# christoskokas/gtsam-vSLAM

Measured on AMD Instinct MI355X. Metric: frames/sec (extract+match+localBA), 1500 feat stereo 752x480, higher is better.
Workload: dtype u8/i32 (extract, match) + f64 (pose LM, local BA)

## Files before the change

### gtsam-vslam_amd/csrc/ba.hip

```cpp
#include "common.hpp"
#include "comm.hpp"
#include "dmath.hpp"
#include "ba_pool.hpp"
#include <algorithm>
#include <cmath>
#include <numeric>
#include <vector>
#include <atomic>
#include <condition_variable>
#include <functional>
#include <memory>
#include <mutex>
#include <thread>

namespace vslam {

struct BaEdge {
    int a, b, fa, fb;
    DPose measured;
    double r[6], Ja[36], Jb[36];
    double Haa[36], Hab[36], Hbb[36], ga[6], gb[6];
};

struct BaDev {
    int NF, Lp, F, K, NE, n;
    const int* facKf; const int* facFi; const int* facLp; const int* facLm;
    const double* facZ; const double* facIs; const uint8_t* facRight;
    double* facJ;
    const int* lpStart; const int* lpSlotStart; const int* slotStart; const int* slotFi; const int* lpOrig;
    DPose* poseCur; DPose* poseTrial; const int* fidx;
    double* lmCur; double* lmTrial;
    BaEdge* edges;
    double* S; double* rhs; double* Spart; double* Sedge; double* dP; double* dL;
    double* sums; double* partial;
    int* flags;
    double fx, fy, cx, cy, b;
// ... 557 lines not shown
        const double2* src = (const double2*)(D.facJ + (size_t)f0 * 20);
        double2* dst = (double2*)g.F;
        for (int i = lane; i < nf * 10; i += 64) dst[i] = src[i];
        for (int i = lane; i < nf; i += 64) g.ffi[i] = D.facFi[f0 + i];
        for (int i = lane; i <= ns; i += 64) { g.sst[i] = D.slotStart[s0 + i] - f0; g.sfi[i] = D.slotFi[s0 + i]; }
    }
    ba_wave_fence();
    {
        double acc = 0;
        if (R.hOn)
            for (int f = R.hq; f < nf; f += 4) {
                const double* o = g.F + f * 20;
                acc += o[R.hx] * o[R.hy] + o[R.hx + 3] * o[R.hy + R.hyStep];
            }
        acc += ba2_dpp_xor(acc, 0);
        acc += ba2_dpp_xor(acc, 1);
        if (R.hOn && R.hq == 0) g.hb[R.hk] = R.hSign * acc;
    }
    ba_wave_fence();
#pragma unroll
    for (int k = 0; k < 9; k++) h[k] = g.hb[k];
}
__device__ __forceinline__ void ba2_w_row(const Ba2Region& g, const Ba2Roles& R, double& w0, double& w1, double& w2) {
    w0 = w1 = w2 = 0;
    for (int f = g.sst[R.ws]; f < g.sst[R.ws + 1]; f++) {
        const double* o = g.F + f * 20;
        const double a0 = o[2 + R.wi], a1 = o[8 + R.wi];
        w0 += a0 * o[14] + a1 * o[17];
        w1 += a0 * o[15] + a1 * o[18];
        w2 += a0 * o[16] + a1 * o[19];
    }
}

__global__ __launch_bounds__(1024) void k_ba_schur2(const BaDev* __restrict__ tab, int maxSlots, int maxFac) {
    BaDev D = *lane_entry(tab, blockIdx.z);
    extern __shared__ double sm[];
    if (!ba_enter(D, BA_TRY, blockIdx.y)) return;
    const int n = D.n;
    const int sys = n * n + n;
    double* const Sloc = sm;
    double* const racc = Sloc + (size_t)n * n;
    const int lane = threadIdx.x & 63;
    const int unit = __builtin_amdgcn_readfirstlane(threadIdx.x >> 6), nu = blockDim.x >> 6, nt = blockDim.x;
    const Ba2Region g = ba2_region(sm + sys + (size_t)unit * ba2_stage_doubles(maxFac, maxSlots), maxFac, maxSlots);
    double* const F = g.F; double* const W = g.W; double* const WH = g.WH;
    int* const ffi = g.ffi; int* const sfi = g.sfi;
    const double lam = D.lambda;
    Ba2Roles R;
    R.init(lane);
    const int pf = lane / 6, pi = lane - pf * 6;
    for (int i = threadIdx.x; i < sys; i += nt) Sloc[i] = 0;
    __syncthreads();
    for (int lp = blockIdx.x * nu + unit; lp < D.Lp; lp += gridDim.x * nu) {
        double h[9];
        int nf, ns;
        ba2_stage_h(D, lp, g, R, lane, h, nf, ns);
        double Hi[9];
        ba_hll_inverse(h, lam, Hi);
        if (R.ws < ns) {
            double w0, w1, w2;
            ba2_w_row(g, R, w0, w1, w2);
            const double g0 = w0 * Hi[0] + w1 * Hi[3] + w2 * Hi[6], g1 = w0 * Hi[1] + w1 * Hi[4] + w2 * Hi[7], g2 = w0 * Hi[2] + w1 * Hi[5] + w2 * Hi[8];
            double* wr = W + R.ws * 18 + R.wi * 3;
            wr[0] = w0; wr[1] = w1; wr[2] = w2;
            double* gr = WH + R.ws * 18 + R.wi * 3;
            gr[0] = g0; gr[1] = g1; gr[2] = g2;
            atomicAdd(&racc[6 * sfi[R.ws] + R.wi], -(g0 * h[6] + g1 * h[7] + g2 * h[8]));
        }
        ba_wave_fence();
        {
            const int nb = ns * (ns + 1) / 2, half = lane & 1;
            for (int b0 = 0; b0 < nb; b0 += 32) {
                int b = b0 + (lane >> 1), s1 = 0;
                if (b >= nb) continue;
                while (b >= ns - s1) { b -= ns - s1; s1++; }
                const int s2 = s1 + b;
                const double* A = WH + s1 * 18 + half * 9;
                const double* B = W + s2 * 18;
                double bb[18];
#pragma unroll
                for (int q = 0; q < 18; q++) bb[q] = B[q];
                double* d0 = Sloc + (6 * sfi[s1] + 3 * half) * n + 6 * sfi[s2];
#pragma unroll
                for (int i = 0; i < 3; i++) {
                    const double a0 = A[3 * i], a1 = A[3 * i + 1], a2 = A[3 * i + 2];
                    double* dr = d0 + i * n;
#pragma unroll
                    for (int j = 0; j < 6; j++) atomicAdd(dr + j, -(a0 * bb[3 * j] + a1 * bb[3 * j + 1] + a2 * bb[3 * j + 2]));
                }
            }
        }
        if (pf < 10)
            for (int fb = 0; fb < nf; fb += 10) {
                const int f = fb + pf;
                if (f >= nf) break;
                const int fi = ffi[f];
                if (fi < 0) continue;
                const double* o = F + f * 20;
                const double a0 = o[2 + pi], a1 = o[8 + pi];
                double* dr = Sloc + (6 * fi + pi) * n + 6 * fi;
                for (int j = pi; j < 6; j++) atomicAdd(dr + j, a0 * o[2 + j] + a1 * o[8 + j]);
                atomicAdd(&racc[6 * fi + pi], -(a0 * o[0] + a1 * o[1]));
            }
        ba_wave_fence();
    }
    __syncthreads();
    double* dst = D.Spart + (size_t)blockIdx.x * sys;
    for (int i = threadIdx.x; i < sys; i += nt) dst[i] = Sloc[i];
}

__global__ __launch_bounds__(512) void k_ba_back2(const BaDev* __restrict__ tab, int maxSlots, int maxFac) {
    BaDev D = *lane_entry(tab, blockIdx.z);
    extern __shared__ double sm[];
    if (!ba_enter(D, BA_TRY, 0)) return;
    const int nc = D.nAct;
    const int sel = ((const int*)(D.ctl + CTL_INTS))[CI_SEL];
    const int lane = threadIdx.x & 63;
    const int unit = __builtin_amdgcn_readfirstlane(threadIdx.x >> 6), nu = blockDim.x >> 6;
    const Ba2Region g = ba2_region(sm + (size_t)unit * ba2_stage_doubles(maxFac, maxSlots), maxFac, maxSlots);
    Ba2Roles R;
    R.init(lane);
    for (int lp = blockIdx.x * nu + unit; lp < D.Lp; lp += gridDim.x * nu) {
        double h[9];
        int nf, ns;
        ba2_stage_h(D, lp, g, R, lane, h, nf, ns);
        double w0 = 0, w1 = 0, w2 = 0;
        int kcol = 0;
        if (R.ws < ns) { ba2_w_row(g, R, w0, w1, w2); kcol = 6 * g.sfi[R.ws] + R.wi; }
        const int l = D.lpOrig[lp];
        double lamk = D.lambda;
        for (int k = 0; k < nc; k++, lamk *= 10.0) {
            const double* dPk = D.dP + (size_t)k * D.n;
            const double dp = R.ws < ns ? dPk[kcol] : 0.0;
            double t0 = w0 * dp, t1 = w1 * dp, t2 = w2 * dp;
            t0 += ba2_dpp_xor(t0, 0); t1 += ba2_dpp_xor(t1, 0); t2 += ba2_dpp_xor(t2, 0);
            t0 += ba2_dpp_xor(t0, 1); t1 += ba2_dpp_xor(t1, 1); t2 += ba2_dpp_xor(t2, 1);
#pragma unroll
            for (int d = 4; d <= 32; d <<= 1) { t0 += __shfl_xor(t0, d); t1 += __shfl_xor(t1, d); t2 += __shfl_xor(t2, d); }
            double Hi[9];
            ba_hll_inverse(h, lamk, Hi);
            if (lane < 3) {
                const double u0 = h[6] - t0, u1 = h[7] - t1, u2 = h[8] - t2;
                const double h0 = lane == 0 ? Hi[0] : (lane == 1 ? Hi[3] : Hi[6]);
                const double h1 = lane == 0 ? Hi[1] : (lane == 1 ? Hi[4] : Hi[7]);
                const double h2 = lane == 0 ? Hi[2] : (lane == 1 ? Hi[5] : Hi[8]);
                const double dl = h0 * u0 + h1 * u1 + h2 * u2;
                D.dL[(size_t)k * D.dLStride + 3 * (size_t)lp + lane] = dl;
                double* lmT = D.lmBase + (size_t)ba_slot(sel, k, D.NB) * D.lmStride;
                lmT[3 * (size_t)l + lane] = D.lmCur[3 * (size_t)l + lane] + dl;
            }
        }
        ba_wave_fence();
    }
}

__global__ __launch_bounds__(256) void k_ba_reduce(const BaDev* __restrict__ tab, int nPart) {
    BaDev D = *lane_entry(tab, blockIdx.z);
    __shared__ double sSl[8][33];
    if (!ba_enter(D, BA_TRY, blockIdx.y)) return;
    const int total = D.n * D.n + D.n;
    const int e = threadIdx.x & 31, y = threadIdx.x >> 5;
    const int i = blockIdx.x * 32 + e;
    const size_t stride = (size_t)total;
    double s = 0;
    if (i < total) {
        const int per = (nPart + 7) / 8;
        const int p0 = y * per, p1 = min(nPart, p0 + per);
        double s0 = 0, s1 = 0, s2 = 0, s3 = 0;
        int p = p0;
        for (; p + 3 < p1; p += 4) {
            s0 += D.Spart[(size_t)p * stride + i];
            s1 += D.Spart[(size_t)(p + 1) * stride + i];
            s2 += D.Spart[(size_t)(p + 2) * stride + i];
            s3 += D.Spart[(size_t)(p + 3) * stride + i];
        }
        for (; p < p1; p++) s0 += D.Spart[(size_t)p * stride + i];
        s = (s0 + s1) + (s2 + s3);
    }
    sSl[y][e] = s;
    __syncthreads();
    if (y == 0 && i < total) {
        double t = D.Sedge[i];
        for (int q = 0; q < 8; q++) t += sSl[q][e];
        if (D.specLin) D.Sedge2[i] = 0;
        if (i < D.n * D.n) D.S[i] = t; else D.rhs[i - D.n * D.n] = t;
    }
}

struct BaWin {
    int TB, T, TP, tileDoubles, nWin;
    const int* winA; const int* winB;
    const int* winFirstWg;
    const int* wgWin; const int* wgBegin; const int* wgEnd;
    const int* winLm;
    double* part;
    double* Wg; double* Hg;
};

constexpr int BA_WIN_HG = 9 + 6 * BA_MAX_NB;
__global__ __launch_bounds__(64 * BA_SCHUR_WAVES) void k_ba_lm_prep(const BaDev* __restrict__ tab, BaWin Wn, int maxSlots) {
    BaDev D = *lane_entry(tab, blockIdx.z);
    extern __shared__ int smi[];
    if (!ba_enter(D, BA_TRY, 0)) return;
    constexpr int BA_LPL = 64;
    const int lane = threadIdx.x & 63, unit = threadIdx.x >> 6, nu = blockDim.x >> 6;
    int* sfi = smi + unit * maxSlots;
    for (int lp = blockIdx.x * nu + unit; lp < D.Lp; lp += gridDim.x * nu) {
        double h[9];
        int ns = 0;
        ba_lm_blocks<BA_LPL>(D, lp, true, Wn.Wg + (size_t)D.lpSlotStart[lp] * 18, sfi, h, ns);
        double* Hl = Wn.Hg + (size_t)lp * BA_WIN_HG;
        if (lane < 9) {
            double v = h[0];
#pragma unroll
            for (int k = 1; k < 9; k++) if (lane == k) v = h[k];
            Hl[lane] = v;
        } else if (lane >= 16 && lane < 16 + D.nAct) {
            double lamk = D.lambda;
// ... 1557 lines not shown
                    h_facIs[f] = 1.0 / (1.0 / (double)P->inv_sigma_factor[P->pair_octave[2 * p + side]]);
                    h_facRight[f] = (uint8_t)side;
                    h_facPair[f] = p;
                }
                h_slotStart[se] = f1; h_slotFi[se] = -1;
            }
        });
        h_lpSlotStart[Lp] = nSlotEntries;
        for (int l = 0; l < L; l++) h_lmPresent[l] = T.lmPresent[l];
        fill_small(P, T, pose0, edgeSlots);
    }
    void fill_small(const vslam_ba_problem* P, BaHostTmp& T, const DPose* pose0, int edgeSlots) {
        const int K = P->n_kf;
        for (int k = 0; k < K; k++) { h_fidx[k] = T.fidx[k]; h_kfPresent[k] = T.kfPresent[k]; }
        for (int i = 0; i < NE; i++) {
            BaEdge e{};
            e.a = T.order[i]; e.b = T.order[i + 1]; e.fa = T.fidx[e.a]; e.fb = T.fidx[e.b];
            DPose ai;
            pose_inverse(pose0[e.a], ai);
            pose_compose(ai, pose0[e.b], e.measured);
            for (int sl = 0; sl < edgeSlots; sl++) h_edges[(size_t)sl * NE + i] = e;
        }
    }
};

static vslam_status ba_kernel_attributes() {
    static std::once_flag once;
    static hipError_t err = hipSuccess;
    static bool reserveOk = true;
    std::call_once(once, [] {
        const int cap = BA_LDS_BYTES;
        const void* fns[] = {(const void*)k_ba_schur, (const void*)k_ba_schur_win, (const void*)k_ba_solve, (const void*)k_ba_back,
                             (const void*)k_ba_solve_mfma, (const void*)k_ba_chol_col, (const void*)k_ba_chol_back, (const void*)k_ba_lm_prep,
                             (const void*)k_ba_schur2, (const void*)k_ba_back2};
        const void* batchFns[] = {(const void*)k_ba_schur, (const void*)k_ba_schur2, (const void*)k_ba_back, (const void*)k_ba_back2, (const void*)k_ba_solve_mfma};
        for (const void* f : fns) {
            hipFuncAttributes fa{};
            hipError_t e = hipFuncGetAttributes(&fa, f);
            if (e == hipSuccess) e = hipFuncSetAttribute(f, hipFuncAttributeMaxDynamicSharedMemorySize, cap - (int)fa.sharedSizeBytes);
            if (e != hipSuccess && err == hipSuccess) err = e;
            for (const void* b : batchFns) if (b == f && e == hipSuccess && fa.sharedSizeBytes > (size_t)BA_STATIC_LDS_RESERVE) reserveOk = false;
        }
    });
    if (err != hipSuccess) { set_error("hipFuncSetAttribute(MaxDynamicSharedMemorySize): %s", hipGetErrorString(err)); return VSLAM_ERR_HIP; }
    if (!reserveOk) { set_error("local BA: a batch kernel's static LDS exceeds BA_STATIC_LDS_RESERVE"); return VSLAM_ERR_CAPACITY; }
    return VSLAM_OK;
}

static vslam_status ba_run(const vslam_ba_problem* P, vslam_ba_result* R, int device, const vslam_comm* comm) {
#ifdef VSLAM_HOST_STAMPS
    const double bhs_fn0 = bhs_now();
#endif
#ifndef VSLAM_HOST_STAMPS
    auto bhs_t = std::chrono::steady_clock::now();
    g_bhsCalls++;
#endif
    if (!P || !R || P->n_kf < 1 || P->n_lm < 0 || P->n_pairs < 0 || P->n_levels < 1 || P->n_levels > MAX_LEVELS ||
        !P->kf_pose_wc || !P->kf_id || !P->kf_fixed || !P->kf_local || !P->sigma_factor || !P->inv_sigma_factor ||
        !R->kf_pose_wc || !R->lm_xyz || !R->pair_wrong ||
        (P->n_lm > 0 && !P->lm_xyz) ||
        (P->n_pairs > 0 && (!P->pair_kf || !P->pair_lm || !P->pair_flags || !P->pair_uv || !P->pair_octave))) {
        set_error("vslam_local_ba: invalid problem");
        return VSLAM_ERR_INVALID;
    }
    const int rank = comm ? comm->rank : 0, world = comm ? comm->world : 1;
    int ndev = 0;
    if (hipGetDeviceCount(&ndev) != hipSuccess || ndev <= 0) { set_error("no HIP device available (no CPU fallback)"); return VSLAM_ERR_NO_DEVICE; }
    if (device < 0 || device >= ndev) return VSLAM_ERR_INVALID;
// ... 461 lines not shown
        const BaDev* const dD = A.dev(h_D);
        VS_HIP(hipMemcpyAsync((void*)dD, h_D, sizeof(BaDev), hipMemcpyHostToDevice, stream));
        BHS("upload");

        auto run_lm = [&](int ps, long long nfStat, long long lpStat, long long k2Stat) -> vslam_status {
        (void)poseOut; (void)lmOut;
        const int fuseCtl = comm ? 0 : 1;
        const int facBlocks = (NF ? obsBlocks : 0) + std::max(NE, 1);
        const int nObs = NF ? obsBlocks : 0;
        VS_HIP(hipMemsetAsync(d_Sedge.p, 0, ((size_t)n * n + n) * sizeof(double), stream));
        auto step = [&](bool first) -> vslam_status {
            int t = -1;
            if (first || !specLin) {
                t = g_baTimer.begin("ba_linearize");
                hipLaunchKernelGGL(k_ba_factors<0>, dim3(facBlocks), dim3(256), 0, stream, dD, nObs, fuseCtl, relTol, absTol);
                g_baTimer.end(t);
            }
            if (comm) {
                const int tc = g_baTimer.begin("ba_allreduce"); VS_CHECK(comm_allreduce(comm, d_sums.p, 1, stream)); g_baTimer.end(tc);
                hipLaunchKernelGGL(k_ba_ctl, dim3(1), dim3(256), 0, stream, dD, 0, relTol, absTol);
            }
            t = g_baTimer.begin("ba_schur");
            if (n > 0) {
                if (ldsS) hipLaunchKernelGGL(k_ba_schur, dim3(lmBlocks, sharedW ? 1 : NB), dim3(64 * schurWaves), schurLds, stream, dD, maxSlots, sharedW);
                else if (nWinWg) {
                    hipLaunchKernelGGL(k_ba_lm_prep, dim3(std::max(1, std::min((Lp + BA_SCHUR_WAVES - 1) / BA_SCHUR_WAVES, 4 * nCU))), dim3(64 * BA_SCHUR_WAVES),
                                       (size_t)BA_SCHUR_WAVES * maxSlots * sizeof(int), stream, dD, Wn, maxSlots);
                    hipLaunchKernelGGL(k_ba_schur_win, dim3(nWinWg), dim3(64 * schurWaves), schurLds, stream, dD, Wn);
                }
            }
            g_baTimer.end(t);
            t = g_baTimer.begin("ba_solve");
            if (n > 0) {
                if (ldsS) hipLaunchKernelGGL(k_ba_reduce, dim3(((int)sysDoubles + 31) / 32, NB), dim3(256), 0, stream, dD, lmBlocks);
                else hipLaunchKernelGGL(k_ba_reduce_win, dim3(Wn.nWin, NB), dim3(256), 0, stream, dD, Wn);
            }
            if (comm && n > 0) { const int tc = g_baTimer.begin("ba_allreduce"); VS_CHECK(comm_allreduce(comm, d_S.p, sysStride * (NB - 1) + (size_t)n * n + n, stream)); g_baTimer.end(tc); }
            if (n <= 64 && useMfma) hipLaunchKernelGGL(k_ba_solve_mfma64, dim3(NB), dim3(64), 0, stream, dD);
            else if (n <= BA_WAVE_N) hipLaunchKernelGGL(k_ba_solve_wave, dim3(NB), dim3(64), 0, stream, dD);
            else if (n <= BA_MFMA_N && useMfma) hipLaunchKernelGGL(k_ba_solve_mfma, dim3(NB), dim3(64 * BA_MFMA_NW), mfmaLds, stream, dD, d_Lg.p);
            else if (useChol) {
                for (int J = 0; J < cholN / CH_B; J++)
                    hipLaunchKernelGGL(k_ba_chol_col, dim3(cholN / CH_B - J, NB), dim3(256), cholColLds, stream, dD, d_Lg.p, d_cholY.p, cholN, J, d_cholFail.p);
                hipLaunchKernelGGL(k_ba_chol_back, dim3(NB), dim3(256), cholBackLds, stream, dD, (const double*)d_Lg.p, (const double*)d_cholY.p, cholN, d_cholFail.p);
            } else hipLaunchKernelGGL(k_ba_solve, dim3(NB), dim3(std::max(64, vslam::align_up(n, 64))),
                                    solveLds ? solveLdsBytes : 64, stream, dD, solveLds ? 1 : 0, solveLds ? ldA : n);
            g_baTimer.end(t);
            t = g_baTimer.begin("ba_back");
            if (Lp) hipLaunchKernelGGL(k_ba_back, dim3(backBlocks, sharedBack ? 1 : NB), dim3(64 * backWaves), backLds, stream, dD, maxSlots, sharedBack);
            g_baTimer.end(t);
            t = g_baTimer.begin("ba_eval");
            hipLaunchKernelGGL(k_ba_factors<1>, dim3(facBlocks, NB), dim3(256), 0, stream, dD, nObs, fuseCtl, relTol, absTol);
            g_baTimer.end(t);
            if (comm) {
                const int tc = g_baTimer.begin("ba_allreduce"); VS_CHECK(comm_allreduce(comm, d_sums.p + SUMS_CAND, (size_t)2 * NB, stream)); g_baTimer.end(tc);
                hipLaunchKernelGGL(k_ba_ctl, dim3(1), dim3(256), 0, stream, dD, 1, relTol, absTol);
            }
            VS_HIP(hipGetLastError());
            return VSLAM_OK;
        };
        double* h_ctlOut = ws->h_ctlOut;
        const int* co = (const int*)(h_ctlOut + CTL_INTS);
        int enq = 0;
        for (;;) {
            static const int perPoll = getenv("VSLAM_BA_STEPS_PER_POLL") ? std::max(1, atoi(getenv("VSLAM_BA_STEPS_PER_POLL"))) : 4;
            for (int b = 0; b < perPoll; b++) VS_CHECK(step(enq + b == 0));
            enq += perPoll;
// ... 121 lines not shown
                if (!devOrder) for (int l = 0; l < L; l++) h_lmPresent[l] = lmP2[l];
                init_ctl(1);
                VS_HIP(hipMemcpyAsync(A.dev(h_kfPresent), h_kfPresent, K, hipMemcpyHostToDevice, stream));
                if (devOrder) VS_HIP(hipMemcpyAsync(A.dev(h_lmPresent), O.lmPres, (size_t)L, hipMemcpyDeviceToDevice, stream));
                else if (L) VS_HIP(hipMemcpyAsync(A.dev(h_lmPresent), h_lmPresent, L, hipMemcpyHostToDevice, stream));
                VS_HIP(hipMemcpyAsync(A.dev(h_ctl), h_ctl, CTL_DOUBLES * sizeof(double), hipMemcpyHostToDevice, stream));
                if (NF) hipLaunchKernelGGL(k_ba_mask, dim3((NF + 255) / 256), dim3(256), 0, stream, NF, A.dev(h_facPair), d_wrong.p, A.dev(h_facIs));
                {
                    const int nPose = K * (int)(sizeof(DPose) / sizeof(double)), nLm = 3 * L;
                    hipLaunchKernelGGL(k_ba_init_slots, dim3((std::max(nPose, nLm) + 255) / 256, nSlots), dim3(256), 0, stream,
                                       nPose, (const double*)p_pose0, (double*)d_poseS.p, nLm, p_lm0, d_lmS.p);
                }
                VS_CHECK(run_lm(1, NF2, Lp2, k2));
                break;
            }
        }
    }
    BHS("chi2");
    BHS("fetch");
    if (!resultFetched) {
        VS_HIP(hipMemcpyAsync(poseOut, poseFinal, K * sizeof(DPose), hipMemcpyDeviceToHost, stream));
        if (L) VS_HIP(hipMemcpyAsync(lmOut, lmFinal, (size_t)3 * L * sizeof(double), hipMemcpyDeviceToHost, stream));
        VS_HIP(hipStreamSynchronize(stream));
    }
    for (int k = 0; k < K; k++) pose_to_rm16(poseOut[k], R->kf_pose_wc + 16 * (size_t)k);
    if (L) memcpy(R->lm_xyz, lmOut, (size_t)3 * L * sizeof(double));
    if (NP) memcpy(R->pair_wrong, wrong.data(), NP);
    return VSLAM_OK;
}

static std::atomic<long long> g_bbsNs[12], g_bbsCalls{0}, g_bbsPolls{0};
static const char* g_bbsName[12] = {"check+count", "arena fill", "tables+upload", "lm pass 1", "chi2 1", "second-pass prep", "lm pass 2", "chi2 2 + fetch", "results", nullptr, nullptr, nullptr};

struct BaPlanKnobs { bool schur2, back2, sharedW; int s2Waves, b2Waves, schurWaves, lmBlocks; };
static BaPlanKnobs ba_plan_knobs() {
    static const bool s2Env = !(getenv("VSLAM_BA_SCHUR2") && atoi(getenv("VSLAM_BA_SCHUR2")) == 0);
    static const bool b2Env = !(getenv("VSLAM_BA_BACK2") && atoi(getenv("VSLAM_BA_BACK2")) == 0);
    BaPlanKnobs k;
    k.schur2 = s2Env; k.back2 = b2Env;
    k.sharedW = getenv("VSLAM_BA_SCHUR_SHARED") ? atoi(getenv("VSLAM_BA_SCHUR_SHARED")) != 0 : true;
    k.schurWaves = getenv("VSLAM_BA_SCHUR_WAVES_B") ? atoi(getenv("VSLAM_BA_SCHUR_WAVES_B")) : 0;
    k.lmBlocks = getenv("VSLAM_BA_LMBLOCKS") ? atoi(getenv("VSLAM_BA_LMBLOCKS")) : 0;
    k.s2Waves = getenv("VSLAM_BA_SCHUR2_WAVES") ? atoi(getenv("VSLAM_BA_SCHUR2_WAVES")) : 8;
    k.b2Waves = getenv("VSLAM_BA_BACK2_WAVES") ? atoi(getenv("VSLAM_BA_BACK2_WAVES")) : 4;
    return k;
}
static inline int ba_batch_solve_kind(int n, bool useMfma) { return (n <= 64 && useMfma) ? BA_SOLVE_MFMA64 : n <= BA_WAVE_N ? BA_SOLVE_WAVE : BA_SOLVE_MFMA; }
static inline bool ba_batch_single(const vslam_ba_lane_shape& s, bool useMfma) {
    return s.own_rig || s.n_free_kf > BA_LDS_MAX_F || s.n_free_kf <= 0 || s.n_factors <= 0 || s.n_pairs <= 0 || (!useMfma && 6 * s.n_free_kf > BA_WAVE_N);
}
static void ba_batch_plan(const vslam_ba_batch_shape& S, const BaPlanKnobs& kn, vslam_ba_batch_plan& p) {
    p = vslam_ba_batch_plan{};
    const int NB = std::max(1, std::min((int)BA_MAX_NB, (int)S.lookahead));
    const bool useMfma = S.solver == 0;
    p.status = VSLAM_OK; p.lookahead = NB;
    int maxSlots = 1, maxFac = 1, fMax = 0, lpMax = 0, NL = 0;
    for (int i = 0; i < S.n_lanes; i++) {
        const vslam_ba_lane_shape& s = S.lanes[i];
        if (ba_batch_single(s, useMfma)) { p.n_single++; continue; }
        NL++;
        maxSlots = std::max(maxSlots, (int)s.max_slots); maxFac = std::max(maxFac, (int)s.max_factors);
        fMax = std::max(fMax, (int)s.n_free_kf); lpMax = std::max(lpMax, (int)s.n_points);
        p.solve_kinds |= 1 << ba_batch_solve_kind(6 * s.n_free_kf, useMfma);
    }
    p.n_batch = NL; p.f_max = fMax; p.max_slots = maxSlots; p.max_factors = maxFac; p.lp_max = lpMax;
    if (NL == 0) { p.solve_kinds = 0; return; }
    const int nCU = 256, nMax = 6 * fMax;
    const size_t sysMax = (size_t)nMax * nMax + nMax;
    constexpr int SCHUR_LPW = 64 / BA_LPL_SCHUR, BACK_LPW = 64 / BA_LPL_BACK;
    auto stage_lds = [&](int nw) { return (size_t)nw * SCHUR_LPW * 2 * maxSlots * 18 * sizeof(double) + (size_t)nw * SCHUR_LPW * maxSlots * sizeof(int) + 16; };
    auto schur_lds = [&](int nw, int copies) { return copies * sysMax * sizeof(double) + stage_lds(nw); };
    int sharedW = 0, schurWaves = BA_SCHUR_WAVES;
    if (NB > 1 && kn.sharedW) for (int nw : {16, 12, 8, 6, 4, 2}) if (schur_lds(nw, NB) <= 150 * 1024) { sharedW = 1; schurWaves = nw; break; }
    if (!sharedW) { if (kn.schurWaves) schurWaves = kn.schurWaves; while (schurWaves > 2 && schur_lds(schurWaves, 1) > 150 * 1024) schurWaves /= 2; }
    const size_t schurLds = schur_lds(schurWaves, sharedW ? NB : 1);
    const int schurUnits = schurWaves * SCHUR_LPW;
    int lmBlocks = std::max(1, std::min((lpMax + schurUnits - 1) / schurUnits, kn.lmBlocks ? kn.lmBlocks : std::max(16, 2 * nCU / NL)));
    const size_t s2StageB = (size_t)ba2_stage_doubles(maxFac, maxSlots) * sizeof(double);
    int s2Waves = std::max(2, std::min(16, kn.s2Waves));
    while (s2Waves > 2 && sysMax * sizeof(double) + s2Waves * s2StageB > 156 * 1024) s2Waves /= 2;
    const size_t s2Lds = sysMax * sizeof(double) + (size_t)s2Waves * s2StageB;
    const bool useSchur2 = kn.schur2 && fMax <= BA2_MAX_F && maxSlots <= BA2_MAX_F && s2Lds <= 156 * 1024;
    if (useSchur2) lmBlocks = std::max(1, std::min((lpMax + 2 * s2Waves - 1) / (2 * s2Waves), kn.lmBlocks ? kn.lmBlocks : std::max(4, (16 / s2Waves) * nCU / NL)));
    int b2Waves = std::max(1, std::min(8, kn.b2Waves));
    while (b2Waves > 1 && (size_t)b2Waves * s2StageB > BA_DYN_LDS_MAX) b2Waves /= 2;
    const size_t b2Lds = (size_t)b2Waves * s2StageB;
    const bool useBack2 = useSchur2 && kn.back2 && b2Lds <= BA_DYN_LDS_MAX;
    int backWaves = BA_SCHUR_WAVES / BACK_LPW;
    auto back_lds = [&](int nw) { return (size_t)nw * BACK_LPW * maxSlots * 18 * sizeof(double) + (size_t)nw * BACK_LPW * maxSlots * sizeof(int) + 16; };
    while (backWaves > 1 && back_lds(backWaves) > 150 * 1024) backWaves /= 2;
    p.schur_kernel = useSchur2 ? VSLAM_BA_KERNEL_SCHUR2 : VSLAM_BA_KERNEL_SCHUR;
    p.schur_waves = useSchur2 ? s2Waves : schurWaves;
    p.schur_shared_w = useSchur2 ? 0 : sharedW;
    p.schur_blocks = lmBlocks;
    p.schur_lds = (int)(useSchur2 ? s2Lds : schurLds);
    p.back_kernel = useBack2 ? VSLAM_BA_KERNEL_BACK2 : VSLAM_BA_KERNEL_BACK;
    if (useBack2) {
        p.back_waves = b2Waves; p.back_shared = 1; p.back_lds = (int)b2Lds;
        p.back_blocks = std::max(1, std::min((lpMax + 2 * b2Waves - 1) / (2 * b2Waves), std::max(8, (16 / b2Waves) * nCU / NL)));
    } else {
        p.back_waves = backWaves; p.back_shared = NB > 1 ? 1 : 0; p.back_lds = (int)back_lds(backWaves);
        p.back_blocks = std::max(1, std::min((lpMax + backWaves * BACK_LPW - 1) / (backWaves * BACK_LPW), std::max(16, 2 * nCU / NL)));
    }
    p.solve_lds = (p.solve_kinds & (1 << BA_SOLVE_MFMA)) ? (int)(((size_t)BA_MFMA_N * BA_MFMA_LD + 16 + BA_MFMA_N) * sizeof(double)) : 0;
    if (p.schur_lds > BA_DYN_LDS_MAX || p.back_lds > BA_DYN_LDS_MAX || p.solve_lds > BA_DYN_LDS_MAX) p.status = VSLAM_ERR_CAPACITY;
}
thread_local vslam_ba_batch_plan g_baLastPlan{};

static vslam_status ba_run_batch(const vslam_ba_problem* const* Ps, vslam_ba_result* const* Rs, int N, int device) {
    g_baLastPlan = vslam_ba_batch_plan{};
    if (N <= 0 || !Ps || !Rs) return VSLAM_ERR_INVALID;
    if (N == 1) { g_baLastPlan.n_single = 1; return ba_run(Ps[0], Rs[0], device, nullptr); }
    auto bbs_t = std::chrono::steady_clock::now();
    g_bbsCalls++;
    auto BBS = [&](int k) { const auto t_ = std::chrono::steady_clock::now(); g_bbsNs[k] += std::chrono::duration_cast<std::chrono::nanoseconds>(t_ - bbs_t).count(); bbs_t = t_; };
    int ndev = 0;
    if (hipGetDeviceCount(&ndev) != hipSuccess || ndev <= 0) { set_error("no HIP device available (no CPU fallback)"); return VSLAM_ERR_NO_DEVICE; }
    if (device < 0 || device >= ndev) return VSLAM_ERR_INVALID;
    VS_HIP(hipSetDevice(device));
    struct BatchWs {
        hipStream_t stream = nullptr; int device = -1;
        PinnedArena arena;
        DevBuf<uint8_t> d_mem;
        uint8_t* h_back = nullptr; size_t backCap = 0;
        BaPool pool;
        void release() {
            if (device < 0 || hipSetDevice(device) != hipSuccess) return;
            if (stream) { hipStreamSynchronize(stream); hipStreamDestroy(stream); }
// ... 107 lines not shown
    if (fits) {
        uint8_t* pp = h_present;
        for (int a = 0; a < NL; a++) { Lane& q = lanes[act[a]]; q.H.h_kfPresent = pp; pp += q.K; q.H.h_lmPresent = pp; pp += std::max(q.L, 1); }
    }
    if (!fits) { set_error("local BA batch: upload arena too small"); return VSLAM_ERR_CAPACITY; }
    W.pool.run(NL, [&](int a) {
        Lane& q = lanes[act[a]];
        const vslam_ba_problem* P = q.P;
        memcpy(q.h_pose0, q.pose0.data(), (size_t)q.K * sizeof(DPose));
        if (q.L) memcpy(q.h_lm0, P->lm_xyz, (size_t)3 * q.L * sizeof(double));
        memcpy(q.h_pairKf, P->pair_kf, (size_t)q.NP * 4); memcpy(q.h_pairLm, P->pair_lm, (size_t)q.NP * 4);
        memcpy(q.h_pairOct, P->pair_octave, (size_t)2 * q.NP * 4); memcpy(q.h_pairFlags, P->pair_flags, q.NP);
        memcpy(q.h_pairUv, P->pair_uv, (size_t)4 * q.NP * 4); memcpy(q.h_kfLocal, P->kf_local, q.K);
        q.H.fill(P, q.wrong.data(), 0, 1, q.T, q.pose0.data(), nullptr, nSlots);
        ba_init_ctl(q.H.h_ctl, 0, adaptive ? 1 : NB);
    });
    BBS(1);
    int nMax = 0, neMax = 0, nfMax = 0, npMax = 0, valMax = 0;
    for (int i : act) {
        const Lane& q = lanes[i];
        nMax = std::max(nMax, q.H.n); neMax = std::max(neMax, q.H.NE);
        nfMax = std::max(nfMax, q.H.NF); npMax = std::max(npMax, q.NP);
        valMax = std::max(valMax, std::max(q.K * (int)(sizeof(DPose) / sizeof(double)), 3 * q.L));
    }
    plan_cohort();
    const vslam_ba_batch_plan& plan = g_baLastPlan;
    if (plan.status != VSLAM_OK) { set_error("local BA batch: landmark with too many views for the LDS staging"); return VSLAM_ERR_CAPACITY; }
    const int nCU = 256;
    const int obsBlocks = std::max(1, std::min((nfMax + 255) / 256, std::max(16, 2 * nCU / NL)));
    const int facBlocks = obsBlocks + std::max(neMax, 1);
    const size_t sysMax = (size_t)nMax * nMax + nMax;
    const int maxSlots = plan.max_slots, maxFac = plan.max_factors, lmBlocks = plan.schur_blocks;
    const bool useSchur2 = plan.schur_kernel == VSLAM_BA_KERNEL_SCHUR2, useBack2 = plan.back_kernel == VSLAM_BA_KERNEL_BACK2;
    const bool anyMfma64 = plan.solve_kinds & (1 << BA_SOLVE_MFMA64), anyWave = plan.solve_kinds & (1 << BA_SOLVE_WAVE),
               anyMfma = plan.solve_kinds & (1 << BA_SOLVE_MFMA);
    VS_CHECK(ba_kernel_attributes());
    size_t dBytes = 0;
    auto dtake = [&](size_t bytes) { const size_t at = dBytes; dBytes = (dBytes + std::max<size_t>(bytes, 8) + 255) & ~(size_t)255; return at; };
    struct Off { size_t flags, sedge, poseS, lmS, facJ, dP, dL, S, partial, spart, sums, Lg, wrong, outPose, outLm; };
    std::vector<Off> off(NL);
    for (int a = 0; a < NL; a++) { const Lane& q = lanes[act[a]]; off[a].flags = dtake(16 * sizeof(int)); off[a].sedge = dtake(((size_t)q.H.n * q.H.n + q.H.n) * nSlots * 8); }
    const size_t zeroBytes = dBytes;
    size_t wrongBase = 0, wrongEnd = 0, outBase = 0, outEnd = 0;
    wrongBase = dBytes;
    for (int a = 0; a < NL; a++) off[a].wrong = dtake(lanes[act[a]].NP);
    wrongEnd = dBytes;
    outBase = dBytes;
    for (int a = 0; a < NL; a++) { const Lane& q = lanes[act[a]]; off[a].outPose = dtake((size_t)q.K * sizeof(DPose)); off[a].outLm = dtake((size_t)3 * q.L * 8); }
    outEnd = dBytes;
    for (int a = 0; a < NL; a++) {
        const Lane& q = lanes[act[a]];
        const BaPassHost& H = q.H;
        const size_t sysStride = (size_t)H.n * H.n + 2 * H.n + 8, sysD = (size_t)H.n * H.n + H.n;
        off[a].poseS = dtake((size_t)nSlots * q.K * sizeof(DPose)); off[a].lmS = dtake((size_t)nSlots * 3 * q.L * 8);
        off[a].facJ = dtake((size_t)20 * H.NF * nSlots * 8); off[a].dP = dtake((size_t)NB * H.n * 8); off[a].dL = dtake((size_t)NB * 3 * H.Lp * 8);
        off[a].S = dtake(sysStride * NB * 8); off[a].partial = dtake(((size_t)2 * obsBlocks + 2 * (size_t)std::max(H.NE, 1)) * NB * 8);
        off[a].spart = dtake(sysD * lmBlocks * NB * 8); off[a].sums = dtake(32 * 8);
        off[a].Lg = (H.n > 64 || !useMfma) && H.n > BA_WAVE_N ? dtake((size_t)BA_MFMA_N * BA_MFMA_N * NB * 8) : 0;
    }
    VS_HIP(W.d_mem.alloc(dBytes));
    uint8_t* const dm = W.d_mem.p;
    const size_t oBackCtl = 0, oBackWrong = ((size_t)CTL_DOUBLES * 8 * NL + 255) & ~(size_t)255, oBackOut = oBackWrong + (wrongEnd - wrongBase);
    const size_t backBytes = oBackOut + (outEnd - outBase);
    if (backBytes > W.backCap) {
        VS_HIP(hipStreamSynchronize(stream));
        if (W.h_back) hipHostFree(W.h_back);
        W.backCap = 2 * backBytes + 4096;
        VS_HIP(hipHostMalloc((void**)&W.h_back, W.backCap, hipHostMallocDefault));
    }
    for (int a = 0; a < NL; a++) {
        Lane& q = lanes[act[a]];
        const BaPassHost& H = q.H;
        const vslam_ba_problem* P = q.P;
        const Off& o = off[a];
        q.d_flags = (int*)(dm + o.flags); q.d_Sedge = (double*)(dm + o.sedge); q.d_poseS = (DPose*)(dm + o.poseS); q.d_lmS = (double*)(dm + o.lmS);
        q.d_facJ = (double*)(dm + o.facJ); q.d_dP = (double*)(dm + o.dP); q.d_dL = (double*)(dm + o.dL); q.d_S = (double*)(dm + o.S);
        q.d_partial = (double*)(dm + o.partial); q.d_Spart = (double*)(dm + o.spart); q.d_sums = (double*)(dm + o.sums);
        q.d_Lg = o.Lg ? (double*)(dm + o.Lg) : nullptr; q.oWrong = oBackWrong + (o.wrong - wrongBase); q.oOut = oBackOut + (o.outPose - outBase);
        q.d_wrong = W.h_back + q.oWrong; q.d_outPose = (double*)(W.h_back + q.oOut);
        q.d_outLm = (double*)(W.h_back + q.oOut + (o.outLm - o.outPose));
        BaDev D{};
        const int n = H.n, K = q.K, L = q.L;
        D.NF = H.NF; D.Lp = H.Lp; D.F = H.F; D.K = K; D.NE = H.NE; D.n = n;
        D.facKf = A.dev(H.h_facKf); D.facFi = A.dev(H.h_facFi); D.facLp = A.dev(H.h_facLp); D.facLm = A.dev(H.h_facLm);
        D.facZ = A.dev(H.h_facZ); D.facIs = A.dev(H.h_facIs); D.facRight = A.dev(H.h_facRight); D.facJ = q.d_facJ;
        D.lpStart = A.dev(H.h_lpStart); D.lpSlotStart = A.dev(H.h_lpSlotStart); D.slotStart = A.dev(H.h_slotStart); D.slotFi = A.dev(H.h_slotFi);
        D.lpOrig = A.dev(H.h_lpOrig); D.poseCur = q.d_poseS; D.poseTrial = q.d_poseS + K; D.fidx = A.dev(H.h_fidx);
        D.lmCur = q.d_lmS; D.lmTrial = q.d_lmS + (size_t)3 * L; D.edges = A.dev(H.h_edges);
        D.S = q.d_S; D.rhs = q.d_S + (size_t)n * n; D.Sedge = q.d_Sedge; D.dP = q.d_dP; D.dL = q.d_dL; D.sums = q.d_sums; D.flags = q.d_flags;
        D.fx = P->rig.fx; D.fy = P->rig.fy; D.cx = P->rig.cx; D.cy = P->rig.cy; D.b = (double)P->rig.baseline;
        D.ctl = A.dev(H.h_ctl);
        D.NB = NB; D.specLin = 1; D.adaptive = adaptive ? 1 : 0;
        D.poseBase = q.d_poseS; D.lmBase = q.d_lmS; D.lmStride = (size_t)3 * L;
        D.facJBase = q.d_facJ; D.facJStride = (size_t)20 * H.NF; D.SedgeBase = q.d_Sedge; D.edgesBase = A.dev(H.h_edges);
        D.sysStride = (size_t)n * n + 2 * n + 8; D.dLStride = (size_t)3 * H.Lp;
        D.partialStride = (size_t)2 * obsBlocks + 2 * (size_t)std::max(H.NE, 1); D.partial = q.d_partial;
        D.spartStride = ((size_t)n * n + n) * lmBlocks; D.Spart = q.d_Spart;
        D.solveKind = ba_batch_solve_kind(n, useMfma);
        D.Lg = q.d_Lg;
        D.ctlHost = (double*)(W.h_back + oBackCtl) + (size_t)CTL_DOUBLES * a;
        *H.h_D = D;
        BaLaneAux X{};
        X.C.NP = q.NP; X.C.pairKf = A.dev(q.h_pairKf); X.C.pairLm = A.dev(q.h_pairLm); X.C.pairFlags = A.dev(q.h_pairFlags); X.C.pairUv = A.dev(q.h_pairUv);
        X.C.pairOct = A.dev(q.h_pairOct); X.C.kfLocal = A.dev(q.h_kfLocal); X.C.kfPresent = A.dev(H.h_kfPresent); X.C.lmPresent = A.dev(H.h_lmPresent);
        X.C.wrong = q.d_wrong;
        for (int l = 0; l < P->n_levels; l++) X.C.thr[l] = (float)((double)7.815f * (double)P->sigma_factor[l]);
        X.C.fx = D.fx; X.C.fy = D.fy; X.C.cx = D.cx; X.C.cy = D.cy; X.C.b = D.b;
        X.NF = H.NF; X.facPair = A.dev(H.h_facPair); X.facIs = A.dev(H.h_facIs);
        X.nPose = K * (int)(sizeof(DPose) / sizeof(double)); X.nLm = 3 * L; X.pose0 = (const double*)A.dev(q.h_pose0); X.lm0 = A.dev(q.h_lm0);
        X.outPose = q.d_outPose; X.outLm = q.d_outLm;
        h_aux[a] = X;
    }
    const BaDev* const dTab = A.dev(h_tab);
    const BaLaneAux* const dAux = A.dev(h_aux);
    VS_HIP(A.upload(stream));
    VS_HIP(hipMemsetAsync(dm, 0, zeroBytes, stream));
    const int valBlocks = std::max(1, std::min((valMax + 255) / 256, 64));
    hipLaunchKernelGGL(k_ba_init_slots_b, dim3(valBlocks, NL), dim3(256), 0, stream, dTab, dAux);

    auto step = [&](bool first) -> vslam_status {
        int t = -1;
        if (first) {
            t = g_baTimer.begin("ba_linearize");
            hipLaunchKernelGGL(k_ba_factors<0>, dim3(facBlocks, 1, NL), dim3(256), 0, stream, dTab, obsBlocks, 1, relTol, absTol);
            g_baTimer.end(t);
        }
        t = g_baTimer.begin("ba_schur");
        if (useSchur2) hipLaunchKernelGGL(k_ba_schur2, dim3(lmBlocks, NB, NL), dim3(64 * plan.schur_waves), plan.schur_lds, stream, dTab, maxSlots, maxFac);
        else hipLaunchKernelGGL(k_ba_schur, dim3(lmBlocks, plan.schur_shared_w ? 1 : NB, NL), dim3(64 * plan.schur_waves), plan.schur_lds, stream, dTab, maxSlots, plan.schur_shared_w);
        g_baTimer.end(t);
        t = g_baTimer.begin("ba_solve");
        hipLaunchKernelGGL(k_ba_reduce, dim3(((int)sysMax + 31) / 32, NB, NL), dim3(256), 0, stream, dTab, lmBlocks);
        if (anyMfma64) hipLaunchKernelGGL(k_ba_solve_mfma64, dim3(NB, 1, NL), dim3(64), 0, stream, dTab);
        if (anyWave) hipLaunchKernelGGL(k_ba_solve_wave, dim3(NB, 1, NL), dim3(64), 0, stream, dTab);
        if (anyMfma) hipLaunchKernelGGL(k_ba_solve_mfma, dim3(NB, 1, NL), dim3(64 * BA_MFMA_NW), plan.solve_lds, stream, dTab, (double*)nullptr);
        g_baTimer.end(t);
        t = g_baTimer.begin("ba_back");
        if (useBack2) hipLaunchKernelGGL(k_ba_back2, dim3(plan.back_blocks, 1, NL), dim3(64 * plan.back_waves), plan.back_lds, stream, dTab, maxSlots, maxFac);
        else hipLaunchKernelGGL(k_ba_back, dim3(plan.back_blocks, plan.back_shared ? 1 : NB, NL), dim3(64 * plan.back_waves), plan.back_lds, stream, dTab, maxSlots, plan.back_shared);
        g_baTimer.end(t);
        t = g_baTimer.begin("ba_eval");
        hipLaunchKernelGGL(k_ba_factors<1>, dim3(facBlocks, NB, NL), dim3(256), 0, stream, dTab, obsBlocks, 1, relTol, absTol);
        g_baTimer.end(t);
        VS_HIP(hipGetLastError());
        return VSLAM_OK;
    };
    double* const b_ctl = (double*)(W.h_back + oBackCtl);
    memcpy(b_ctl, h_ctlAll, (size_t)CTL_DOUBLES * 8 * NL);
    auto lm_loop = [&](int first) -> vslam_status {
        static const int perPollEnv = getenv("VSLAM_BA_STEPS_PER_POLL") ? std::max(1, atoi(getenv("VSLAM_BA_STEPS_PER_POLL"))) : 0;
        int enq = 0, polls = 0;
        for (;;) {
            const int batch = perPollEnv ? perPollEnv : (enq == 0 ? first : 2);
            for (int b = 0; b < batch; b++) VS_CHECK(step(enq + b == 0));
            enq += batch;
            static const bool mirrorOff = getenv("VSLAM_BA_CTL_MIRROR") && atoi(getenv("VSLAM_BA_CTL_MIRROR")) == 0;
            if (mirrorOff || ++polls > 4) VS_HIP(hipMemcpyAsync(b_ctl, A.dev(h_ctlAll), (size_t)CTL_DOUBLES * 8 * NL, hipMemcpyDeviceToHost, stream));
            VS_HIP(vslam::stream_wait_blocking(stream));
            g_bbsPolls++;
            bool all = true;
            for (int a = 0; a < NL; a++) all &= ((const int*)(b_ctl + (size_t)CTL_DOUBLES * a + CTL_INTS))[CI_STATE] == BA_DONE;
            if (all) return VSLAM_OK;
            if (enq > 400) {
                (void)hipMemcpy(b_ctl, A.dev(h_ctlAll), (size_t)CTL_DOUBLES * 8 * NL, hipMemcpyDeviceToHost);
                for (int a = 0; a < NL; a++) {
// ... 345 lines not shown
```

Before: 29160.

## Accumulate Schur complement in packed upper-triangular block layout in LDS

The schur2 kernel now stores the reduced camera system as packed upper-triangular 6x6 blocks, each padded to a pitch of 37 doubles, instead of a dense n×n row-major matrix. This cuts the LDS footprint of each block, which should help occupancy, reduces the per-block partials written to global memory, and aims to spread the atomics over more LDS banks. The reduce kernel gains a packed mode that maps packed offsets, and the lower-triangle blocks, back to row-major S and rhs. A row-major variant with a padded leading dimension stays selectable through an environment variable, and the block product is restructured to keep fewer values in registers.

```diff
diff --git a/gtsam-vslam_amd/csrc/ba.hip b/gtsam-vslam_amd/csrc/ba.hip
--- a/gtsam-vslam_amd/csrc/ba.hip
+++ b/gtsam-vslam_amd/csrc/ba.hip
@@ -2,6 +2,7 @@
 #include "comm.hpp"
 #include "dmath.hpp"
 #include "ba_pool.hpp"
+#include "ba_packed.hpp"
 #include <algorithm>
 #include <cmath>
 #include <numeric>
@@ -625,18 +626,57 @@
     }
 }
 
-__global__ __launch_bounds__(1024) void k_ba_schur2(const BaDev* __restrict__ tab, int maxSlots, int maxFac) {
+enum { BA2_ROWMAJOR = 0, BA2_ROWMAJOR1 = 1, BA2_PACKED = 2 };
+__host__ __device__ inline int ba2_sys_doubles(int n, int layout) {
+    return layout == BA2_PACKED ? (ba_packed_doubles(n / 6) + 1) & ~1 : layout == BA2_ROWMAJOR1 ? n * (n + 1) + n : n * n + n;
+}
+__host__ __device__ inline int ba2_part_doubles(int n, int layout) {
+    return layout == BA2_PACKED ? ba_packed_doubles(n / 6) : n * n + n;
+}
+template <bool PACKED>
+__device__ __forceinline__ void ba2_blocks(double* Sloc, const double* W, const double* WH, const int* sfi, int ns, int lane, int F, int ld) {
+    const int nb = ns * (ns + 1) / 2, half = lane & 1;
+    for (int b0 = 0; b0 < nb; b0 += 32) {
+        int b = b0 + (lane >> 1), s1 = 0;
+        if (b >= nb) continue;
+        while (b >= ns - s1) { b -= ns - s1; s1++; }
+        const int s2 = s1 + b;
+        const double* A = WH + s1 * 18 + half * 9;
+        const double* B = W + s2 * 18;
+        double aa[9];
+#pragma unroll
+        for (int q = 0; q < 9; q++) aa[q] = A[q];
+        double* d0 = Sloc + (PACKED ? ba_packed_block(F, sfi[s1], sfi[s2]) * BA_PACKED_PITCH + 18 * half : (6 * sfi[s1] + 3 * half) * ld + 6 * sfi[s2]);
+#pragma unroll
+        for (int jh = 0; jh < 2; jh++) {
+            double bb[9];
+#pragma unroll
+            for (int q = 0; q < 9; q++) bb[q] = B[9 * jh + q];
+#pragma unroll
+            for (int i = 0; i < 3; i++) {
+                double* dr = d0 + i * (PACKED ? 6 : ld) + 3 * jh;
+#pragma unroll
+                for (int j = 0; j < 3; j++) atomicAdd(dr + j, -(aa[3 * i] * bb[3 * j] + aa[3 * i + 1] * bb[3 * j + 1] + aa[3 * i + 2] * bb[3 * j + 2]));
+            }
+        }
+    }
+}
+
+template <bool PACKED>
+__device__ __forceinline__ void ba2_schur(const BaDev* __restrict__ tab, int maxSlots, int maxFac, int layout) {
     BaDev D = *lane_entry(tab, blockIdx.z);
     extern __shared__ double sm[];
     if (!ba_enter(D, BA_TRY, blockIdx.y)) return;
-    const int n = D.n;
-    const int sys = n * n + n;
+    const int n = D.n, F = n / 6;
+    constexpr bool packed = PACKED;
+    const int ld = layout == BA2_ROWMAJOR1 ? n + 1 : n;
+    const int sys = ba2_sys_doubles(n, layout);
     double* const Sloc = sm;
-    double* const racc = Sloc + (size_t)n * n;
+    double* const racc = Sloc + (packed ? ba_packed_rhs(F) : ld * n);
     const int lane = threadIdx.x & 63;
     const int unit = __builtin_amdgcn_readfirstlane(threadIdx.x >> 6), nu = blockDim.x >> 6, nt = blockDim.x;
     const Ba2Region g = ba2_region(sm + sys + (size_t)unit * ba2_stage_doubles(maxFac, maxSlots), maxFac, maxSlots);
-    double* const F = g.F; double* const W = g.W; double* const WH = g.WH;
+    double* const F_ = g.F; double* const W = g.W; double* const WH = g.WH;
     int* const ffi = g.ffi; int* const sfi = g.sfi;
     const double lam = D.lambda;
     Ba2Roles R;
@@ -661,46 +701,32 @@
             atomicAdd(&racc[6 * sfi[R.ws] + R.wi], -(g0 * h[6] + g1 * h[7] + g2 * h[8]));
         }
         ba_wave_fence();
-        {
-            const int nb = ns * (ns + 1) / 2, half = lane & 1;
-            for (int b0 = 0; b0 < nb; b0 += 32) {
-                int b = b0 + (lane >> 1), s1 = 0;
-                if (b >= nb) continue;
-                while (b >= ns - s1) { b -= ns - s1; s1++; }
-                const int s2 = s1 + b;
-                const double* A = WH + s1 * 18 + half * 9;
-                const double* B = W + s2 * 18;
-                double bb[18];
-#pragma unroll
-                for (int q = 0; q < 18; q++) bb[q] = B[q];
-                double* d0 = Sloc + (6 * sfi[s1] + 3 * half) * n + 6 * sfi[s2];
-#pragma unroll
-                for (int i = 0; i < 3; i++) {
-                    const double a0 = A[3 * i], a1 = A[3 * i + 1], a2 = A[3 * i + 2];
-                    double* dr = d0 + i * n;
-#pragma unroll
-                    for (int j = 0; j < 6; j++) atomicAdd(dr + j, -(a0 * bb[3 * j] + a1 * bb[3 * j + 1] + a2 * bb[3 * j + 2]));
-                }
-            }
-        }
+        ba2_blocks<PACKED>(Sloc, W, WH, sfi, ns, lane, F, ld);
         if (pf < 10)
             for (int fb = 0; fb < nf; fb += 10) {
                 const int f = fb + pf;
                 if (f >= nf) break;
                 const int fi = ffi[f];
                 if (fi < 0) continue;
-                const double* o = F + f * 20;
+                const double* o = F_ + f * 20;
                 const double a0 = o[2 + pi], a1 = o[8 + pi];
-                double* dr = Sloc + (6 * fi + pi) * n + 6 * fi;
+                double* dr = Sloc + (packed ? ba_packed_block(F, fi, fi) * BA_PACKED_PITCH + 6 * pi : (6 * fi + pi) * ld + 6 * fi);
                 for (int j = pi; j < 6; j++) atomicAdd(dr + j, a0 * o[2 + j] + a1 * o[8 + j]);
                 atomicAdd(&racc[6 * fi + pi], -(a0 * o[0] + a1 * o[1]));
             }
         ba_wave_fence();
     }
     __syncthreads();
-    double* dst = D.Spart + (size_t)blockIdx.x * sys;
-    for (int i = threadIdx.x; i < sys; i += nt) dst[i] = Sloc[i];
-}
+    const int part = ba2_part_doubles(n, layout);
+    double* dst = D.Spart + (size_t)blockIdx.x * part;
+    if (layout == BA2_ROWMAJOR1) {
+        for (int i = threadIdx.x; i < part; i += nt) dst[i] = Sloc[i + i / n];
+    } else {
+        for (int i = threadIdx.x; i < part; i += nt) dst[i] = Sloc[i];
+    }
+}
+__global__ __launch_bounds__(1024) void k_ba_schur2(const BaDev* __restrict__ tab, int maxSlots, int maxFac) { ba2_schur<true>(tab, maxSlots, maxFac, BA2_PACKED); }
+__global__ __launch_bounds__(1024) void k_ba_schur2_rm(const BaDev* __restrict__ tab, int maxSlots, int maxFac, int layout) { ba2_schur<false>(tab, maxSlots, maxFac, layout); }
 
 __global__ __launch_bounds__(512) void k_ba_back2(const BaDev* __restrict__ tab, int maxSlots, int maxFac) {
     BaDev D = *lane_entry(tab, blockIdx.z);
@@ -747,36 +773,41 @@
     }
 }
 
-__global__ __launch_bounds__(256) void k_ba_reduce(const BaDev* __restrict__ tab, int nPart) {
+__global__ __launch_bounds__(256) void k_ba_reduce(const BaDev* __restrict__ tab, int nPart, int packed) {
     BaDev D = *lane_entry(tab, blockIdx.z);
     __shared__ double sSl[8][33];
     if (!ba_enter(D, BA_TRY, blockIdx.y)) return;
-    const int total = D.n * D.n + D.n;
+    const int total = D.n * D.n + D.n, F = D.n / 6;
+    const int nSum = packed ? ba_packed_doubles(F) : total;
+    const int nSlots = packed ? ba_packed_reduce_slots(F) : total;
     const int e = threadIdx.x & 31, y = threadIdx.x >> 5;
     const int i = blockIdx.x * 32 + e;
-    const size_t stride = (size_t)total;
     double s = 0;
-    if (i < total) {
+    if (i < nSum) {
         const int per = (nPart + 7) / 8;
         const int p0 = y * per, p1 = min(nPart, p0 + per);
         double s0 = 0, s1 = 0, s2 = 0, s3 = 0;
         int p = p0;
         for (; p + 3 < p1; p += 4) {
-            s0 += D.Spart[(size_t)p * stride + i];
-            s1 += D.Spart[(size_t)(p + 1) * stride + i];
-            s2 += D.Spart[(size_t)(p + 2) * stride + i];
-            s3 += D.Spart[(size_t)(p + 3) * stride + i];
-        }
-        for (; p < p1; p++) s0 += D.Spart[(size_t)p * stride + i];
+            s0 += D.Spart[p * nSum + i];
+            s1 += D.Spart[(p + 1) * nSum + i];
+            s2 += D.Spart[(p + 2) * nSum + i];
+            s3 += D.Spart[(p + 3) * nSum + i];
+        }
+        for (; p < p1; p++) s0 += D.Spart[p * nSum + i];
         s = (s0 + s1) + (s2 + s3);
     }
     sSl[y][e] = s;
     __syncthreads();
-    if (y == 0 && i < total) {
-        double t = D.Sedge[i];
-        for (int q = 0; q < 8; q++) t += sSl[q][e];
-        if (D.specLin) D.Sedge2[i] = 0;
-        if (i < D.n * D.n) D.S[i] = t; else D.rhs[i - D.n * D.n] = t;
+    const int slot = blockIdx.x * 32 + threadIdx.x;
+    if (y == 0 && slot < nSlots) {
+        const int io = packed ? ba_packed_reduce_entry(F, slot) : slot;
+        if (io >= 0) {
+            double t = D.Sedge[io];
+            for (int q = 0; q < 8; q++) t += sSl[q][threadIdx.x];
+            if (D.specLin) D.Sedge2[io] = 0;
+            if (io < D.n * D.n) D.S[io] = t; else D.rhs[io - D.n * D.n] = t;
+        }
     }
 }
 
@@ -2400,8 +2431,8 @@
         const int cap = BA_LDS_BYTES;
         const void* fns[] = {(const void*)k_ba_schur, (const void*)k_ba_schur_win, (const void*)k_ba_solve, (const void*)k_ba_back,
                              (const void*)k_ba_solve_mfma, (const void*)k_ba_chol_col, (const void*)k_ba_chol_back, (const void*)k_ba_lm_prep,
-                             (const void*)k_ba_schur2, (const void*)k_ba_back2};
-        const void* batchFns[] = {(const void*)k_ba_schur, (const void*)k_ba_schur2, (const void*)k_ba_back, (const void*)k_ba_back2, (const void*)k_ba_solve_mfma};
+                             (const void*)k_ba_schur2, (const void*)k_ba_schur2_rm, (const void*)k_ba_back2};
+        const void* batchFns[] = {(const void*)k_ba_schur, (const void*)k_ba_schur2, (const void*)k_ba_schur2_rm, (const void*)k_ba_back, (const void*)k_ba_back2, (const void*)k_ba_solve_mfma};
         for (const void* f : fns) {
             hipFuncAttributes fa{};
             hipError_t e = hipFuncGetAttributes(&fa, f);
@@ -2929,7 +2960,7 @@
             g_baTimer.end(t);
             t = g_baTimer.begin("ba_solve");
             if (n > 0) {
-                if (ldsS) hipLaunchKernelGGL(k_ba_reduce, dim3(((int)sysDoubles + 31) / 32, NB), dim3(256), 0, stream, dD, lmBlocks);
+                if (ldsS) hipLaunchKernelGGL(k_ba_reduce, dim3(((int)sysDoubles + 31) / 32, NB), dim3(256), 0, stream, dD, lmBlocks, 0);
                 else hipLaunchKernelGGL(k_ba_reduce_win, dim3(Wn.nWin, NB), dim3(256), 0, stream, dD, Wn);
             }
             if (comm && n > 0) { const int tc = g_baTimer.begin("ba_allreduce"); VS_CHECK(comm_allreduce(comm, d_S.p, sysStride * (NB - 1) + (size_t)n * n + n, stream)); g_baTimer.end(tc); }
@@ -3117,7 +3148,7 @@
 static std::atomic<long long> g_bbsNs[12], g_bbsCalls{0}, g_bbsPolls{0};
 static const char* g_bbsName[12] = {"check+count", "arena fill", "tables+upload", "lm pass 1", "chi2 1", "second-pass prep", "lm pass 2", "chi2 2 + fetch", "results", nullptr, nullptr, nullptr};
 
-struct BaPlanKnobs { bool schur2, back2, sharedW; int s2Waves, b2Waves, schurWaves, lmBlocks; };
+struct BaPlanKnobs { bool schur2, back2, sharedW; int s2Waves, b2Waves, schurWaves, lmBlocks, s2Layout; };
 static BaPlanKnobs ba_plan_knobs() {
     static const bool s2Env = !(getenv("VSLAM_BA_SCHUR2") && atoi(getenv("VSLAM_BA_SCHUR2")) == 0);
     static const bool b2Env = !(getenv("VSLAM_BA_BACK2") && atoi(getenv("VSLAM_BA_BACK2")) == 0);
@@ -3128,6 +3159,7 @@
     k.lmBlocks = getenv("VSLAM_BA_LMBLOCKS") ? atoi(getenv("VSLAM_BA_LMBLOCKS")) : 0;
     k.s2Waves = getenv("VSLAM_BA_SCHUR2_WAVES") ? atoi(getenv("VSLAM_BA_SCHUR2_WAVES")) : 8;
     k.b2Waves = getenv("VSLAM_BA_BACK2_WAVES") ? atoi(getenv("VSLAM_BA_BACK2_WAVES")) : 4;
+    k.s2Layout = getenv("VSLAM_BA_SCHUR2_LAYOUT") ? std::max(0, std::min((int)BA2_PACKED, atoi(getenv("VSLAM_BA_SCHUR2_LAYOUT")))) : (int)BA2_PACKED;
     return k;
 }
 static inline int ba_batch_solve_kind(int n, bool useMfma) { return (n <= 64 && useMfma) ? BA_SOLVE_MFMA64 : n <= BA_WAVE_N ? BA_SOLVE_WAVE : BA_SOLVE_MFMA; }
@@ -3178,7 +3210,7 @@
     p.schur_waves = useSchur2 ? s2Waves : schurWaves;
     p.schur_shared_w = useSchur2 ? 0 : sharedW;
     p.schur_blocks = lmBlocks;
-    p.schur_lds = (int)(useSchur2 ? s2Lds : schurLds);
+    p.schur_lds = (int)(useSchur2 ? (size_t)ba2_sys_doubles(nMax, kn.s2Layout) * sizeof(double) + (size_t)s2Waves * s2StageB : schurLds);
     p.back_kernel = useBack2 ? VSLAM_BA_KERNEL_BACK2 : VSLAM_BA_KERNEL_BACK;
     if (useBack2) {
         p.back_waves = b2Waves; p.back_shared = 1; p.back_lds = (int)b2Lds;
@@ -3352,6 +3384,10 @@
     const size_t sysMax = (size_t)nMax * nMax + nMax;
     const int maxSlots = plan.max_slots, maxFac = plan.max_factors, lmBlocks = plan.schur_blocks;
     const bool useSchur2 = plan.schur_kernel == VSLAM_BA_KERNEL_SCHUR2, useBack2 = plan.back_kernel == VSLAM_BA_KERNEL_BACK2;
+    const int s2Layout = ba_plan_knobs().s2Layout;
+    const bool packedS = useSchur2 && s2Layout == BA2_PACKED;
+    const int reduceSlots = packedS ? ba_packed_reduce_slots(nMax / 6) : (int)sysMax;
+    auto part_doubles = [&](int n) { return (size_t)(useSchur2 ? ba2_part_doubles(n, s2Layout) : n * n + n); };
     const bool anyMfma64 = plan.solve_kinds & (1 << BA_SOLVE_MFMA64), anyWave = plan.solve_kinds & (1 << BA_SOLVE_WAVE),
                anyMfma = plan.solve_kinds & (1 << BA_SOLVE_MFMA);
     VS_CHECK(ba_kernel_attributes());
@@ -3371,11 +3407,11 @@
     for (int a = 0; a < NL; a++) {
         const Lane& q = lanes[act[a]];
         const BaPassHost& H = q.H;
-        const size_t sysStride = (size_t)H.n * H.n + 2 * H.n + 8, sysD = (size_t)H.n * H.n + H.n;
+        const size_t sysStride = (size_t)H.n * H.n + 2 * H.n + 8;
         off[a].poseS = dtake((size_t)nSlots * q.K * sizeof(DPose)); off[a].lmS = dtake((size_t)nSlots * 3 * q.L * 8);
         off[a].facJ = dtake((size_t)20 * H.NF * nSlots * 8); off[a].dP = dtake((size_t)NB * H.n * 8); off[a].dL = dtake((size_t)NB * 3 * H.Lp * 8);
         off[a].S = dtake(sysStride * NB * 8); off[a].partial = dtake(((size_t)2 * obsBlocks + 2 * (size_t)std::max(H.NE, 1)) * NB * 8);
-        off[a].spart = dtake(sysD * lmBlocks * NB * 8); off[a].sums = dtake(32 * 8);
+        off[a].spart = dtake(part_doubles(H.n) * lmBlocks * NB * 8); off[a].sums = dtake(32 * 8);
         off[a].Lg = (H.n > 64 || !useMfma) && H.n > BA_WAVE_N ? dtake((size_t)BA_MFMA_N * BA_MFMA_N * NB * 8) : 0;
     }
     VS_HIP(W.d_mem.alloc(dBytes));
@@ -3415,7 +3451,7 @@
         D.facJBase = q.d_facJ; D.facJStride = (size_t)20 * H.NF; D.SedgeBase = q.d_Sedge; D.edgesBase = A.dev(H.h_edges);
         D.sysStride = (size_t)n * n + 2 * n + 8; D.dLStride = (size_t)3 * H.Lp;
         D.partialStride = (size_t)2 * obsBlocks + 2 * (size_t)std::max(H.NE, 1); D.partial = q.d_partial;
-        D.spartStride = ((size_t)n * n + n) * lmBlocks; D.Spart = q.d_Spart;
+        D.spartStride = part_doubles(n) * lmBlocks; D.Spart = q.d_Spart;
         D.solveKind = ba_batch_solve_kind(n, useMfma);
         D.Lg = q.d_Lg;
         D.ctlHost = (double*)(W.h_back + oBackCtl) + (size_t)CTL_DOUBLES * a;
@@ -3446,11 +3482,12 @@
             g_baTimer.end(t);
         }
         t = g_baTimer.begin("ba_schur");
-        if (useSchur2) hipLaunchKernelGGL(k_ba_schur2, dim3(lmBlocks, NB, NL), dim3(64 * plan.schur_waves), plan.schur_lds, stream, dTab, maxSlots, maxFac);
+        if (useSchur2 && s2Layout == BA2_PACKED) hipLaunchKernelGGL(k_ba_schur2, dim3(lmBlocks, NB, NL), dim3(64 * plan.schur_waves), plan.schur_lds, stream, dTab, maxSlots, maxFac);
+        else if (useSchur2) hipLaunchKernelGGL(k_ba_schur2_rm, dim3(lmBlocks, NB, NL), dim3(64 * plan.schur_waves), plan.schur_lds, stream, dTab, maxSlots, maxFac, s2Layout);
         else hipLaunchKernelGGL(k_ba_schur, dim3(lmBlocks, plan.schur_shared_w ? 1 : NB, NL), dim3(64 * plan.schur_waves), plan.schur_lds, stream, dTab, maxSlots, plan.schur_shared_w);
         g_baTimer.end(t);
         t = g_baTimer.begin("ba_solve");
-        hipLaunchKernelGGL(k_ba_reduce, dim3(((int)sysMax + 31) / 32, NB, NL), dim3(256), 0, stream, dTab, lmBlocks);
+        hipLaunchKernelGGL(k_ba_reduce, dim3((reduceSlots + 31) / 32, NB, NL), dim3(256), 0, stream, dTab, lmBlocks, packedS ? 1 : 0);
         if (anyMfma64) hipLaunchKernelGGL(k_ba_solve_mfma64, dim3(NB, 1, NL), dim3(64), 0, stream, dTab);
         if (anyWave) hipLaunchKernelGGL(k_ba_solve_wave, dim3(NB, 1, NL), dim3(64), 0, stream, dTab);
         if (anyMfma) hipLaunchKernelGGL(k_ba_solve_mfma, dim3(NB, 1, NL), dim3(64 * BA_MFMA_NW), plan.solve_lds, stream, dTab, (double*)nullptr);
diff --git a/gtsam-vslam_amd/csrc/ba_packed.hpp b/gtsam-vslam_amd/csrc/ba_packed.hpp
--- /dev/null
+++ b/gtsam-vslam_amd/csrc/ba_packed.hpp
@@ -0,0 +1,46 @@
+#pragma once
+
+#ifndef BA_PACKED_PITCH
+#define BA_PACKED_PITCH 37
+#endif
+
+#ifndef BA_PACKED_HD
+#if defined(__HIPCC__) || defined(__CUDACC__)
+#define BA_PACKED_HD __host__ __device__ inline
+#else
+#define BA_PACKED_HD inline
+#endif
+#endif
+
+BA_PACKED_HD int ba_packed_blocks(int F) { return F * (F + 1) / 2; }
+BA_PACKED_HD int ba_packed_block(int F, int a, int b) { return a * (2 * F - a + 1) / 2 + (b - a); }
+BA_PACKED_HD int ba_packed_off(int F, int a, int b, int i, int j) { return ba_packed_block(F, a, b) * BA_PACKED_PITCH + 6 * i + j; }
+BA_PACKED_HD int ba_packed_rhs(int F) { return ba_packed_blocks(F) * BA_PACKED_PITCH; }
+BA_PACKED_HD int ba_packed_doubles(int F) { return ba_packed_rhs(F) + 6 * F; }
+BA_PACKED_HD int ba_packed_from_rowmajor(int F, int e) {
+    const int n = 6 * F;
+    if (e >= n * n) return ba_packed_rhs(F) + (e - n * n);
+    const int r = e / n, c = e - r * n, a = r / 6, b = c / 6;
+    if (a > b) return -1;
+    return ba_packed_off(F, a, b, r - 6 * a, c - 6 * b);
+}
+BA_PACKED_HD int ba_packed_to_rowmajor(int F, int off) {
+    const int n = 6 * F, rhs = ba_packed_rhs(F);
+    if (off >= rhs) return n * n + (off - rhs);
+    const int blk = off / BA_PACKED_PITCH, in = off - blk * BA_PACKED_PITCH;
+    if (in >= 36) return -1;
+    int a = 0, first = 0;
+    while (blk >= first + F - a) { first += F - a; a++; }
+    const int b = a + (blk - first), i = in / 6, j = in - 6 * i;
+    return (6 * a + i) * n + 6 * b + j;
+}
+BA_PACKED_HD int ba_packed_reduce_slots(int F) { return ba_packed_doubles(F) + 36 * (F * (F - 1) / 2); }
+BA_PACKED_HD int ba_packed_reduce_entry(int F, int t) {
+    const int size = ba_packed_doubles(F);
+    if (t < size) return ba_packed_to_rowmajor(F, t);
+    const int k = t - size, lb = k / 36, in = k - 36 * lb;
+    int a = 1;
+    while (lb >= a * (a + 1) / 2) a++;
+    const int b = lb - a * (a - 1) / 2, i = in / 6, j = in - 6 * i;
+    return (6 * a + i) * (6 * F) + 6 * b + j;
+}
```

New measurement: 29720 (median of 6 runs). +1.9%, better.
